# urbste/MultiCol-SLAM

Hardware: AMD Instinct MI355X
Metric: Mfeatures/s extract+match, 3-cam 754x480 multi-frame (higher is better)
Workload: dtype u8+i32 (images, Hamming) / f64 (omni model)

## Files before the change

### multicol-slam_amd/csrc/mcs_describe.hip

```cpp
#include "mcs_common.h"
#include <type_traits>
#include "mcs_orient.h"

#include <algorithm>
#include <cstdlib>
#include <vector>

namespace mcs {

__constant__ __attribute__((aligned(16))) signed char c_pattern[2048];

template <int NB> struct UPat;
template <> struct UPat<2> { static constexpr int R = 4, RW = 1; };
template <> struct UPat<4> { static constexpr int R = 6, RW = 2; };
template <> struct UPat<8> { static constexpr int R = 9, RW = 5; };
constexpr int kUPatMax = 9 * 64, kUWMax = 5 * 64;
__device__ double2 g_upat[3][kUPatMax];
__device__ double g_uw[3][kUWMax];
__device__ unsigned short g_gidx[3][64 * 16];

template <int NB>
static bool build_unique_pattern(const signed char* pattern, int slot) {
	constexpr int R = UPat<NB>::R, RW = UPat<NB>::RW, NP = 128 * NB;
	std::vector<int> first, mult, ofPoint(NP);
	for (int i = 0; i < NP; ++i) {
		int f = -1;
		for (size_t k = 0; k < first.size(); ++k)
			if (pattern[2 * first[k]] == pattern[2 * i] && pattern[2 * first[k] + 1] == pattern[2 * i + 1]) { f = (int)k; break; }
		if (f < 0) { f = (int)first.size(); first.push_back(i); mult.push_back(0); }
		mult[f]++; ofPoint[i] = f;
	}
	const int nu = (int)first.size(), pad = R * 64 - nu;
	int heavy = 0;
	for (int m : mult) heavy += m >= 2;
	if (pad < 0 || heavy + pad > RW * 64) return false;
	std::vector<int> order;
	for (int k = 0; k < nu; ++k) if (mult[k] >= 2) order.push_back(k);
	for (int k = 0; k < pad; ++k) order.push_back(-1);
	for (int k = 0; k < nu; ++k) if (mult[k] < 2) order.push_back(k);
	std::vector<int> slotOf(nu);
	std::vector<double2> up(kUPatMax, double2{0.0, 0.0});
	std::vector<double> uw(kUWMax, 0.0);
	for (int sidx = 0; sidx < R * 64; ++sidx) {
		const int k = order[sidx], src = first[k < 0 ? 0 : k];
		up[sidx] = double2{(double)pattern[2 * src], (double)pattern[2 * src + 1]};
		if (k >= 0) slotOf[k] = sidx;
		if (sidx < RW * 64) uw[sidx] = k < 0 ? 0.0 : (double)mult[k];
		else if (k < 0 || mult[k] != 1) return false;
	}
	std::vector<unsigned short> gi(64 * 16, 0);
	for (int l = 0; l < 64; ++l)
		for (int i = 0; i < 2 * NB; ++i) gi[l * 2 * NB + i] = (unsigned short)slotOf[ofPoint[2 * ((i >> 1) * 64 + l) + (i & 1)]];
	return hipMemcpyToSymbol(HIP_SYMBOL(g_upat), up.data(), sizeof(double2) * kUPatMax, sizeof(double2) * kUPatMax * slot) == hipSuccess &&
	       hipMemcpyToSymbol(HIP_SYMBOL(g_uw), uw.data(), sizeof(double) * kUWMax, sizeof(double) * kUWMax * slot) == hipSuccess &&
	       hipMemcpyToSymbol(HIP_SYMBOL(g_gidx), gi.data(), sizeof(unsigned short) * 64 * 16, sizeof(unsigned short) * 64 * 16 * slot) == hipSuccess;
}

bool upload_describe_tables(const signed char* pattern) {
	if (!pattern) return false;
	if (hipMemcpyToSymbol(HIP_SYMBOL(c_pattern), pattern, 2048) != hipSuccess) return false;
	return build_unique_pattern<2>(pattern, 0) && build_unique_pattern<4>(pattern, 1) && build_unique_pattern<8>(pattern, 2);
}

__device__ __forceinline__ double recip_refined(double d) {
	const double r0 = __builtin_amdgcn_rcp(d);
	const double r1 = __builtin_fma(r0, __builtin_fma(-d, r0, 1.0), r0);
	return __builtin_fma(r1, __builtin_fma(-d, r1, 1.0), r1);
}
__device__ __forceinline__ double div_shared(double a, double d, double r) {
	const double q0 = a * r;
	return __builtin_fma(__builtin_fma(-d, q0, a), r, q0);
}

__global__ void k_selftest_recip(unsigned long long seed, int n, int* mismatches) {
	const int i = blockIdx.x * blockDim.x + threadIdx.x;
	if (i >= n) return;
	unsigned long long st = seed + 0x9E3779B97F4A7C15ull * (unsigned long long)(i + 1);
	auto next = [&]() { st ^= st >> 12; st ^= st << 25; st ^= st >> 27; return st * 0x2545F4914F6CDD1Dull; };
	auto unit = [&]() { return (double)(next() >> 11) * (1.0 / 9007199254740992.0); };
	const double ed = -14.0 + 19.0 * unit();
	const double d = exp10(ed) * (1.0 + unit());
	double a = (unit() * 2.0 - 1.0) * exp10(-18.0 + 22.0 * unit());
	if ((i & 127) == 0) a = 0.0;
	if ((i & 127) == 1) a = -d;
	if ((i & 127) == 2) a = d;
	const double r = recip_refined(d);
	const double q1 = div_shared(a, d, r), q2 = a / d;
	if (__double_as_longlong(q1) != __double_as_longlong(q2)) atomicAdd(mismatches, 1);
}

void launch_selftest_recip(unsigned long long seed, int n, int* mismatches, hipStream_t s) {
	hipLaunchKernelGGL(k_selftest_recip, dim3((n + 255) / 256), dim3(256), 0, s, seed, n, mismatches);
}

__device__ __forceinline__ double uniform_f64(const double* p) {
	const unsigned lo = __builtin_amdgcn_readfirstlane(reinterpret_cast<const unsigned*>(p)[0]);
	const unsigned hi = __builtin_amdgcn_readfirstlane(reinterpret_cast<const unsigned*>(p)[1]);
	return __hiloint2double((int)hi, (int)lo);
}

__device__ __forceinline__ double horner_d(const double* coeffs, int s, double x) {
	double c[MCS_MAX_POLY];
#pragma unroll
	for (int i = 0; i < MCS_MAX_POLY; ++i) c[i] = coeffs[i];
	double res = 0.0;
#pragma unroll
	for (int i = MCS_MAX_POLY - 1; i >= 0; i--) res = res * x + c[i];
	(void)s;
	return res;
}

__device__ __forceinline__ void world2img(const OcamDev& cam, double x, double y, double z, double& u, double& v) {
	double norm = sqrt(x * x + y * y);
	if (norm == 0.0) norm = 1e-14;
	const double theta = atan(-z / norm);
	const double rho = horner_d(cam.invP, cam.invP_deg, theta);
	const double uu = x / norm * rho;
	const double vv = y / norm * rho;
	u = uu * cam.c + vv * cam.d + cam.u0;
	v = uu * cam.e + vv + cam.v0;
}

__device__ __forceinline__ void img2world(const OcamDev& cam, double u, double v, double& xo, double& yo, double& zo) {
	const double u_t = u - cam.u0;
	const double v_t = v - cam.v0;
	double x = (u_t - cam.d * v_t) / cam.invAffine;
	double y = (-cam.e * u_t + cam.c * v_t) / cam.invAffine;
	const double X2 = x * x;
	const double Y2 = y * y;
	double z = -horner_d(cam.p, cam.p_deg, sqrt(X2 + Y2));
	double norm = sqrt(X2 + Y2 + z * z);
	xo = x / norm;
	yo = y / norm;
	zo = z / norm;
}

#ifndef MCS_PATCH_R
#define MCS_PATCH_R 21
#endif
constexpr int kPatchR = MCS_PATCH_R, kPatchRows = 2 * kPatchR + 1, kPatchDw = (kPatchRows + 3) / 4, kPatchPitch = 4 * kPatchDw;
constexpr int kPatchBytes = (kPatchRows * kPatchPitch + 15) / 16 * 16;
constexpr int kFPitch = (kPatchRows + 15) / 16 * 16, kFPatchBytes = kPatchRows * kFPitch;

struct Sampler {
	const uint8_t* blur; int bstride;
	const uint8_t* raw; int rstride;
	int w, h;
	const uint8_t* patch; int prow, pcol;
	__device__ __forceinline__ int at(int r, int c) const {
		const unsigned pr = (unsigned)(r - prow), pc = (unsigned)(c - pcol);
		if (pr < (unsigned)kPatchRows && pc < (unsigned)kPatchRows) return patch[pr * kPatchPitch + pc];
		if ((unsigned)r < (unsigned)h && (unsigned)c < (unsigned)w) return blur[(size_t)r * bstride + c];
		r = r < -kEdge ? -kEdge : (r > h + kEdge - 1 ? h + kEdge - 1 : r);
		c = c < -kEdge ? -kEdge : (c > w + kEdge - 1 ? w + kEdge - 1 : c);
		r = r < 0 ? -r : (r >= h ? 2 * (h - 1) - r : r);
		c = c < 0 ? -c : (c >= w ? 2 * (w - 1) - c : c);
		return raw[(size_t)r * rstride + c];
	}
	__device__ __forceinline__ void pair(int row, int col, int dy0, int dx0, int dy1, int dx1, int& t0, int& t1) const {
		const unsigned r0 = (unsigned)(dy0 + kPatchR), c0 = (unsigned)(dx0 + kPatchR), r1 = (unsigned)(dy1 + kPatchR), c1 = (unsigned)(dx1 + kPatchR);
		const bool inside = max(max(r0, c0), max(r1, c1)) < (unsigned)kPatchRows;
		if (!__any(!inside)) {
			t0 = patch[r0 * kPatchPitch + c0];
			t1 = patch[r1 * kPatchPitch + c1];
		} else {
			t0 = at(row + dy0, col + dx0);
			t1 = at(row + dy1, col + dx1);
		}
	}
};

#ifndef MCS_ABLATE
#define MCS_ABLATE 0
#endif
__host__ __device__ constexpr int pat_doubles(int npoints) { return 2 * npoints + 2; }
__host__ __device__ constexpr int coord_bytes(int mode, int npoints) { return mode == 0 ? 0 : pat_doubles(npoints) * 8; }

constexpr int kPatchTrips = (kPatchRows * kPatchDw + 63) / 64;
struct KeyPt {
	int img, out, level, row, col;
	float angle;
	double rayx, rayy, rayz;
	Sampler sm;
};

__device__ __forceinline__ void find_slot(const PyrDesc& d, const int* selCount, int s, int& level, int& pos, int& total) {
	total = 0; level = -1; pos = 0;
	for (int l = 0; l < d.nlevels; ++l) {
		const int c = selCount[l];
		if (s >= total && s < total + c) { level = l; pos = s - total; }
		total += c;
	}
}

__device__ __forceinline__ void patch_load(const uint8_t* blur, int bstride, int row, int col, uint32_t (&pv)[kPatchTrips]) {
	const int lane = threadIdx.x & 63;
	const uint8_t* bp = blur + (size_t)(row - kPatchR) * bstride + (col - kPatchR);
#pragma unroll
	for (int t = 0; t < kPatchTrips; ++t) {
		const int i = min(lane + 64 * t, kPatchRows * kPatchDw - 1);
		const int r = i / kPatchDw, k = i - r * kPatchDw;
		__builtin_memcpy(&pv[t], bp + (size_t)r * bstride + 4 * k, 4);
	}
}
__device__ __forceinline__ void patch_store(uint8_t* patch, const uint32_t (&pv)[kPatchTrips]) {
	const int lane = threadIdx.x & 63;
#pragma unroll
	for (int t = 0; t < kPatchTrips; ++t) {
		const int i = min(lane + 64 * t, kPatchRows * kPatchDw - 1);
		const int r = i / kPatchDw, k = i - r * kPatchDw;
		*reinterpret_cast<uint32_t*>(&patch[r * kPatchPitch + 4 * k]) = pv[t];
	}
}

// ... 388 lines not shown
#pragma unroll
	for (int o = 32; o > 0; o >>= 1) v += __shfl_xor(v, o);
	return v;
}

template <int CTRL>
__device__ __forceinline__ double dpp_f64(double v) {
	const int vl = __double2loint(v), vh = __double2hiint(v);
	const int lo = __builtin_amdgcn_update_dpp(0, vl, CTRL, 0xF, 0xF, true);
	const int hi = __builtin_amdgcn_update_dpp(0, vh, CTRL, 0xF, 0xF, true);
	return __hiloint2double(hi, lo);
}
__device__ __forceinline__ void wave_sum2_f64(double sx, double sy, double& totx, double& toty) {
	const auto l = __builtin_amdgcn_permlane32_swap(__double2loint(sx), __double2loint(sy), false, false);
	const auto h = __builtin_amdgcn_permlane32_swap(__double2hiint(sx), __double2hiint(sy), false, false);
	double z = __hiloint2double((int)h[0], (int)l[0]) + __hiloint2double((int)h[1], (int)l[1]);
	const auto l2 = __builtin_amdgcn_permlane16_swap(__double2loint(z), __double2loint(z), false, false);
	const auto h2 = __builtin_amdgcn_permlane16_swap(__double2hiint(z), __double2hiint(z), false, false);
	z = __hiloint2double((int)h2[0], (int)l2[0]) + __hiloint2double((int)h2[1], (int)l2[1]);
	z += dpp_f64<0x128>(z);
	z += dpp_f64<0x124>(z);
	z += dpp_f64<0x122>(z);
	z += dpp_f64<0x121>(z);
	totx = __hiloint2double(__builtin_amdgcn_readlane(__double2hiint(z), 0), __builtin_amdgcn_readlane(__double2loint(z), 0));
	toty = __hiloint2double(__builtin_amdgcn_readlane(__double2hiint(z), 32), __builtin_amdgcn_readlane(__double2loint(z), 32));
}

struct FastCam { double c, d, e; };
template <class Tab>
__device__ __forceinline__ void fast_w2i(const FastCam& C, Tab tab, double xr, double yr, double& u, double& v, unsigned& top) {
	const double s = __builtin_fma(xr, xr, yr * yr);
	const unsigned hi = (unsigned)__double2hiint(s), lo = (unsigned)__double2loint(s);
	const unsigned idx = (hi >> (20 - kGM)) - (unsigned)((1023 + kGE0) << kGM);
	top = max(top, idx);
	unsigned row = idx < (unsigned)kGRows ? idx : (unsigned)(kGRows - 1);
	if (MCS_FAST_ABLATE & 16) row = 0;
	const double frac = __hiloint2double((int)((hi & ((1u << (20 - kGM)) - 1u)) | 0x3FF00000u), (int)lo);
	const double tau = frac - (1.0 + 1.0 / (double)(2 << kGM));
	typedef double f64x2 __attribute__((ext_vector_type(2)));
	typedef float f32x4 __attribute__((ext_vector_type(4)));
	const auto rowp = reinterpret_cast<const uint8_t*>(tab) + row * (unsigned)kGDevRowBytes;
	const f64x2 g01 = *reinterpret_cast<const f64x2*>(rowp), g23 = *reinterpret_cast<const f64x2*>(rowp + 16);
	const f32x4 g46 = *reinterpret_cast<const f32x4*>(rowp + 32);
	const float tf = (float)tau;
	const float tl = __builtin_fmaf(__builtin_fmaf(g46.z, tf, g46.y), tf, g46.x);
	double G = __builtin_fma((double)tl, tau, g23.y);
	G = __builtin_fma(G, tau, g23.x);
	G = __builtin_fma(G, tau, g01.y);
	G = __builtin_fma(G, tau, g01.x);
	const double uu = xr * G, vv = yr * G;
	u = __builtin_fma(uu, C.c, vv * C.d);
	v = __builtin_fma(uu, C.e, vv);
}

template <int MODE>
__global__ __launch_bounds__(256) void k_orient_b(ExtractBuffers b, int wavesPerImage, int nslots) {
	const int gw = blockIdx.x * 256 + threadIdx.x;
	if (gw >= nslots) return;
	KpAuxSoA A; A.carve(b.aux, nslots);
	const PyrDesc& d = *b.desc;
	const int img = gw / wavesPerImage, s = gw - img * wavesPerImage;
	int total, level, pos;
	find_slot(d, b.selCount + (size_t)img * d.nlevels, s, level, pos, total);
	if (s == 0) {
		b.nkp[img] = total < d.kpCap ? total : d.kpCap;
		if (total > d.kpCap) atomicExch(b.status, MCS_ERR_CAPACITY);
	}
	if (level < 0 || s >= d.kpCap) { A.lvl[gw] = -1; return; }
	const LevelInfo& L = d.lv[level];
	const size_t si = (size_t)img * d.selPerImage + L.selBase + pos;
	const uint32_t rec = b.sel[si];
	const float angle = b.selAngle[si];
	const int col = (int)(rec & 0xFFF) + kMinBorder, row = (int)((rec >> 12) & 0xFFF) + kMinBorder;
	float pxf = (float)col, pyf = (float)row;
	if (level != 0) { pxf = pxf * L.scale; pyf = pyf * L.scale; }
	mcs_keypoint kp;
	kp.x = pxf; kp.y = pyf; kp.size = L.kpSize; kp.angle = angle; kp.response = (float)(rec >> 24); kp.octave = level; kp.class_id = -1;
	b.kps[(size_t)img * d.kpCap + s] = kp;
	A.rc[gw] = row | (col << 16);
	A.poff[gw] = (unsigned)(L.off + (size_t)(row - kPatchR) * L.stride + (col - kPatchR));
	const int lvlWord = level | (L.stride << 16);
	if constexpr (MODE == 0) {
		if (b.cams && b.rays) {
			double rx, ry, rz;
			img2world(b.cams[img], (double)pxf, (double)pyf, rx, ry, rz);
			double* rp = b.rays + ((size_t)img * d.kpCap + s) * 3;
			rp[0] = rx; rp[1] = ry; rp[2] = rz;
		}
		const float DEG2RADf = (float)3.1415926535897932384626433832795 / 180.f;
		const double a0 = (double)(angle * DEG2RADf);
		double* D = A.d8 + gw;
		D[(size_t)2 * nslots] = cos(a0); D[(size_t)3 * nslots] = sin(a0);
		A.lvl[gw] = lvlWord;
		return;
	}
	const OcamDev& cam = b.cams[img];
	double rayx, rayy, rayz;
	img2world(cam, (double)pxf, (double)pyf, rayx, rayy, rayz);
	if (b.rays) {
		double* rp = b.rays + ((size_t)img * d.kpCap + s) * 3;
		rp[0] = rayx; rp[1] = rayy; rp[2] = rayz;
	}
	double ukx = 0.0, uky = 0.0;
	if (d.undistort) {
		const double p0 = cam.p[0];
		ukx = -rayx / rayz * p0;
		uky = -rayy / rayz * p0;
	}
	double* D8 = A.d8 + gw;
	const size_t S = (size_t)nslots;
	D8[0] = ukx; D8[S] = uky;
	const double n2 = ukx * ukx + uky * uky;
	if (cam.fastOk == 0 || !(n2 < 1.0e300)) {
		A.lvl[gw] = lvlWord | kAuxExact;
		b.preList[atomicAdd(b.preCount, 1)] = (uint32_t)gw;
		return;
	}
	A.lvl[gw] = lvlWord;
	double ang[3] = {0.0, 0.0, 0.0};
	if (MODE == 1) {
		const float DEG2RADf = (float)3.1415926535897932384626433832795 / 180.f;
		ang[0] = (double)(angle * DEG2RADf);
	} else {
		const float RHOf = 180.0f / 3.1415926535897932384626f;
		const double RHOd = 180.0 / 3.1415926535897932384626433832795028841971693993;
		const double rot = 20.0 / RHOd;
		ang[0] = (double)(angle / RHOf);
		ang[1] = ang[0] + rot; ang[2] = ang[0] - rot;
	}
#pragma unroll
	for (int k = 0; k < (MODE == 2 ? 3 : 1); ++k) {
		double sn, cs;
		sincos(ang[k], &sn, &cs);
		D8[(2 + 2 * k) * S] = cs; D8[(3 + 2 * k) * S] = sn;
	}
}

#ifndef MCS_FAST_WAVES_PER_EU
#define MCS_FAST_WAVES_PER_EU 4
#endif
#ifndef MCS_FAST_BLOCKS
#define MCS_FAST_BLOCKS (4096 / MCS_FAST_WAVES)
#endif
constexpr int kFastBlocks = MCS_FAST_BLOCKS;
static_assert(kSlotAlign % kFastWaves == 0, "a group's keypoint slots must belong to one image");

struct UTabs {
	const double2* upat; const double* uw; const uint32_t* gidx;
	uint8_t* vals;
};
__host__ __device__ constexpr size_t upat_bytes(int nb) { return (size_t)(nb == 2 ? 4 : nb == 4 ? 6 : 9) * 64 * sizeof(double2); }
__host__ __device__ constexpr size_t uw_bytes(int nb) { return (size_t)(nb == 2 ? 1 : nb == 4 ? 2 : 5) * 64 * sizeof(double); }
__host__ __device__ constexpr size_t gidx_bytes(int nb) { return (size_t)64 * 2 * nb * sizeof(unsigned short); }
__host__ __device__ constexpr size_t uvals_bytes(int nb) { return (size_t)(nb == 2 ? 4 : nb == 4 ? 6 : 9) * 64; }

template <int MODE, int NB, class Ahead>
__device__ __forceinline__ bool fast_keypoint_u(const ExtractBuffers& b, const FastCam& C, const double* tabLds, const uint8_t* patch,
                                                double ukx, double uky, const double (&axc)[3], const double (&ays)[3], const UTabs& T,
                                                unsigned long long (&bitsMain)[NB], unsigned long long (&agree)[NB], Ahead&& ahead) {
	constexpr int NP = 128 * NB, R = UPat<NB>::R, RW = UPat<NB>::RW;
	const double kFix = 1572864.5;
	const unsigned kHiPatch = 0x4137F000u + 4096u - (unsigned)kPatchR;
	const unsigned guardUnits = (unsigned)__builtin_ceil(b.guardEps * 4294967296.0);
	const double gAdd = (double)guardUnits * (1.0 / 4294967296.0);
#pragma unroll
	for (int j = 0; j < NB; ++j) { bitsMain[j] = 0ull; agree[j] = ~0ull; }
	constexpr int npat = MODE == 2 ? 3 : 1;
	typedef double f64x2 __attribute__((ext_vector_type(2)));
	typedef const __attribute__((address_space(3))) f64x2 lds_f64x2;
	typedef const __attribute__((address_space(3))) double lds_f64;
	typedef const __attribute__((address_space(3))) uint32_t lds_u32;
	typedef __attribute__((address_space(3))) uint8_t lds_u8;
	typedef const __attribute__((address_space(3))) uint8_t lds_cu8;
	unsigned pdo = (unsigned)(uintptr_t)(lds_f64x2*)T.upat, pwo = (unsigned)(uintptr_t)(lds_f64*)T.uw, pgo = (unsigned)(uintptr_t)(lds_u32*)T.gidx;
	unsigned pvo = (unsigned)(uintptr_t)(lds_u8*)T.vals, plo = (unsigned)(uintptr_t)(lds_cu8*)patch;
	int lane = threadIdx.x & 63;
	asm volatile("" : "+v"(pdo), "+v"(pwo), "+v"(pgo), "+s"(pvo), "+s"(plo), "+v"(lane));
	lds_f64x2* const pd = (lds_f64x2*)(uintptr_t)pdo;
	lds_f64* const pw = (lds_f64*)(uintptr_t)pwo;
	lds_u32* const pg = (lds_u32*)(uintptr_t)pgo;
	lds_u8* const pv = (lds_u8*)(uintptr_t)pvo;
	lds_cu8* const pvr = (lds_cu8*)(uintptr_t)pvo;
	lds_cu8* const pl = (lds_cu8*)(uintptr_t)plo;
	unsigned top = 0, minlo = 0xFFFFFFFFu, maxrc = 0;
	bool bad = false;
#pragma unroll
	for (int pat = 0; pat < npat; ++pat) {
		const double ax = axc[pat], ay = ays[pat];
		double u[R], v[R];
		double sumx = 0.0, sumy = 0.0;
#pragma unroll
		for (int t = 0; t < R; ++t) {
			const f64x2 p = pd[64 * t];
			if (pat == 0 && t == 0) ahead();
			const double xr = __builtin_fma(p.x, ax, __builtin_fma(-p.y, ay, ukx));
			const double yr = __builtin_fma(p.x, ay, __builtin_fma(p.y, ax, uky));
			if (MCS_FAST_ABLATE & 2) { u[t] = xr; v[t] = yr; } else fast_w2i(C, tabLds, xr, yr, u[t], v[t], top);
			if (t < RW) { const double w = pw[64 * t]; sumx = __builtin_fma(w, u[t], sumx); sumy = __builtin_fma(w, v[t], sumy); }
			else { sumx += u[t]; sumy += v[t]; }
			constexpr int kFence = R > 6 ? 2 : MCS_FAST_FENCE;
			if ((t & (kFence - 1)) == kFence - 1) __builtin_amdgcn_sched_barrier(0);
		}
		double totx, toty;
		wave_sum2_f64(sumx, sumy, totx, toty);
		const double meanX = totx * (1.0 / (double)NP), meanY = toty * (1.0 / (double)NP);
		bad |= !(fabs(meanX) < 16384.0) || !(fabs(meanY) < 16384.0);
		const double cmx = (kFix - meanX) + gAdd, cmy = (kFix - meanY) + gAdd;
		if (R > 6) __builtin_amdgcn_sched_barrier(0);
		int val[R];
#pragma unroll
		for (int t = 0; t < R; ++t) {
			const double yx = u[t] + cmx, yy = v[t] + cmy;
			const unsigned pc = (unsigned)__double2hiint(yx) - kHiPatch, pr = (unsigned)__double2hiint(yy) - kHiPatch;
			if (!(MCS_FAST_ABLATE & 4)) minlo = min(minlo, min((unsigned)__double2loint(yx), (unsigned)__double2loint(yy)));
			maxrc = max(maxrc, max(pr, pc));
			static_assert(kFPitch == 48, "the shift-add form is for a pitch of 48");
			unsigned off16 = (pr << 4) + pc;
			asm volatile("" : "+v"(off16));
			const unsigned offRaw = (pr << 5) + off16;
			const unsigned off = min(offRaw, (unsigned)(kFPatchBytes - 1));
			val[t] = (MCS_FAST_ABLATE & 1) ? (int)off : (int)pl[off];
		}
#pragma unroll
		for (int t = 0; t < R; ++t) pv[64 * t + lane] = (uint8_t)val[t];
		__builtin_amdgcn_fence(__ATOMIC_RELEASE, "wavefront");
#pragma unroll
		for (int j = 0; j < NB; ++j) {
			const uint32_t g = pg[j];
			const int t0 = pvr[g & 0xFFFFu], t1 = pvr[g >> 16];
			const unsigned long long bits = __ballot(t0 < t1);
			if (pat == 0) bitsMain[j] = bits;
			else agree[j] &= ~(bits ^ bitsMain[j]);
		}
		__builtin_amdgcn_fence(__ATOMIC_ACQUIRE, "wavefront");
		if (R > 6) { if (__any(bad | (top >= (unsigned)kGRows) | (minlo < 2u * guardUnits) | (maxrc >= (unsigned)kPatchRows))) return false; }
	}
	bad |= top >= (unsigned)kGRows;
	if (!(MCS_FAST_ABLATE & 4)) bad |= minlo < 2u * guardUnits;
	bad |= maxrc >= (unsigned)kPatchRows;
	return !__any(bad);
}

constexpr int kFastPatchBufs = 2;
constexpr int kMailDwords = 32, kMailBytes = 2 * kMailDwords * 4;
constexpr int kMailCam = 19, kMailUsed = 26;
__host__ __device__ constexpr size_t fast_wave_lds(int nb) { return (size_t)kFastPatchBufs * kFPatchBytes + kMailBytes + uvals_bytes(nb); }
__host__ __device__ constexpr size_t fast_pat_bytes(int nb) { return upat_bytes(nb) + uw_bytes(nb) + gidx_bytes(nb); }

__device__ __forceinline__ unsigned lds_addr(const void* p) { return (unsigned)(uintptr_t)(const __attribute__((address_space(3))) void*)p; }
__device__ __forceinline__ void dma16(const void* g, unsigned ldsBase) {
	asm volatile("s_mov_b32 m0, %1\n\ts_nop 0\n\tglobal_load_lds_dwordx4 %0, off" ::"v"(g), "s"(ldsBase) : "memory", "m0");
}
__device__ __forceinline__ void dma4(const void* g, unsigned ldsBase) {
	asm volatile("s_mov_b32 m0, %1\n\ts_nop 0\n\tglobal_load_lds_dword %0, off" ::"v"(g), "s"(ldsBase) : "memory", "m0");
}
__device__ __forceinline__ void patch_request(const uint8_t* origin, int bstride, uint8_t* patch) {
	int lane = threadIdx.x & 63;
	asm volatile("" : "+v"(lane));
	constexpr int perRow = kFPitch / 16, total = kPatchRows * perRow;
#pragma unroll
	for (int t = 0; t * 64 < total; ++t) {
		const int i = lane + 64 * t;
		const int r = i / perRow, k = i - r * perRow;
		if (64 * (t + 1) <= total || i < total) dma16(origin + (size_t)r * bstride + 16 * k, __builtin_amdgcn_readfirstlane(lds_addr(patch) + 1024 * t));
	}
}
__device__ __forceinline__ void record_request(const KpAuxSoA& A, const OcamDev* cams, int gw, int img, uint32_t* mail) {
	int lane = threadIdx.x & 63;
	asm volatile("" : "+v"(lane));
	const size_t S = (size_t)A.slots;
	const uint32_t* src;
	if (lane < 3) src = reinterpret_cast<const uint32_t*>(A.lvl) + (size_t)lane * S + gw;
	else if (lane < kMailCam) src = reinterpret_cast<const uint32_t*>(A.d8 + (size_t)((lane - 3) >> 1) * S + gw) + ((lane - 3) & 1);
	else if (lane == kMailCam) src = reinterpret_cast<const uint32_t*>(&cams[img].tabIdx);
	else src = reinterpret_cast<const uint32_t*>(&cams[img].c) + (lane - kMailCam - 1);
	if (lane < kMailUsed) dma4(src, __builtin_amdgcn_readfirstlane(lds_addr(mail)));
}
static_assert(offsetof(OcamDev, c) == 0 && offsetof(OcamDev, d) == 8 && offsetof(OcamDev, e) == 16, "record_request reads c, d, e as six consecutive words");

struct FastKp {
	int lvl, rc; unsigned poff; int tabIdx;
	double d8[8]; FastCam C;
	__device__ __forceinline__ bool usable() const { return lvl >= 0 && !(lvl & kAuxExact); }
};
__device__ __forceinline__ int rfl(uint32_t v) { return __builtin_amdgcn_readfirstlane((int)v); }
__device__ __forceinline__ double rfl2(uint32_t lo, uint32_t hi) { return __hiloint2double(rfl(hi), rfl(lo)); }
__device__ __forceinline__ FastKp mail_read(const uint32_t* mail) {
	uint4 q[7];
#pragma unroll
	for (int i = 0; i < 7; ++i) q[i] = reinterpret_cast<const uint4*>(mail)[i];
	const uint32_t* w = reinterpret_cast<const uint32_t*>(q);
	FastKp r;
	r.lvl = rfl(w[0]); r.rc = rfl(w[1]); r.poff = (unsigned)rfl(w[2]); r.tabIdx = rfl(w[kMailCam]);
#pragma unroll
	for (int i = 0; i < 8; ++i) r.d8[i] = rfl2(w[3 + 2 * i], w[4 + 2 * i]);
	r.C.c = rfl2(w[20], w[21]); r.C.d = rfl2(w[22], w[23]); r.C.e = rfl2(w[24], w[25]);
	return r;
}

template <int MODE, int NB>
__attribute__((amdgpu_waves_per_eu(MCS_FAST_WAVES_PER_EU, MCS_FAST_WAVES_PER_EU)))
__global__ __launch_bounds__(64 * kFastWaves) void k_describe_fast(ExtractBuffers b, int wavesPerImage, int nslots, int groupsPerBlock) {
	extern __shared__ __attribute__((aligned(16))) double lds[];
	static_assert(MODE == 1 || MODE == 2, "the fast pass is for the distorted patterns");
	const int wave = __builtin_amdgcn_readfirstlane(threadIdx.x >> 6);
	constexpr size_t kFastWaveLds = fast_wave_lds(NB);
	double2* const patLds = reinterpret_cast<double2*>(reinterpret_cast<uint8_t*>(lds) + kGDevDoubles * sizeof(double));
	uint8_t* const waveLds = reinterpret_cast<uint8_t*>(patLds) + fast_pat_bytes(NB) + (size_t)wave * kFastWaveLds;
	uint32_t* const mailBase = reinterpret_cast<uint32_t*>(waveLds + kFastPatchBufs * kFPatchBytes);
	constexpr int kSlot = NB == 2 ? 0 : NB == 4 ? 1 : 2;
	double* const uwLds = reinterpret_cast<double*>(reinterpret_cast<uint8_t*>(patLds) + upat_bytes(NB));
	uint32_t* const gidxLds = reinterpret_cast<uint32_t*>(reinterpret_cast<uint8_t*>(uwLds) + uw_bytes(NB));
	for (int i = threadIdx.x; i < UPat<NB>::R * 64; i += 64 * kFastWaves) patLds[i] = g_upat[kSlot][i];
	for (int i = threadIdx.x; i < UPat<NB>::RW * 64; i += 64 * kFastWaves) uwLds[i] = g_uw[kSlot][i];
	for (int i = threadIdx.x; i < 64 * NB; i += 64 * kFastWaves) gidxLds[i] = reinterpret_cast<const uint32_t*>(g_gidx[kSlot])[i];
	double* const tabLds = lds;
	const PyrDesc& d = *b.desc;
	KpAuxSoA A; A.carve(b.aux, nslots);
	const int ngroups = nslots / kFastWaves;
	const int nb = (int)gridDim.x, perXcd = (nb + kNumXCD - 1) / kNumXCD;
	const int logical = nb % kNumXCD == 0 ? ((int)blockIdx.x % kNumXCD) * perXcd + (int)blockIdx.x / kNumXCD : (int)blockIdx.x;
	const size_t pyrBytes = d.pyrBytes;
	int curTab = -1;
	auto slot_of = [&](int kk) { const int g = kk * nb + logical; return kk < groupsPerBlock && g < ngroups ? g * kFastWaves + wave : -1; };
	auto ask_record = [&](int kk) { const int gw = slot_of(kk); if (gw >= 0) record_request(A, b.cams, gw, gw / wavesPerImage, mailBase + (kk & 1) * kMailDwords); };
	auto ask_patch = [&](const FastKp& r, int kk) {
		const int gw = slot_of(kk);
		if (gw < 0 || !r.usable()) return;
		patch_request(b.blur + (size_t)(gw / wavesPerImage) * pyrBytes + r.poff, (int)((unsigned)r.lvl >> 16), waveLds + (kk & 1) * kFPatchBytes);
	};
	ask_record(0);
	asm volatile("s_waitcnt vmcnt(0)" ::: "memory");
	FastKp nxt = mail_read(mailBase);
	if (slot_of(0) < 0) nxt.lvl = -1;
	ask_patch(nxt, 0);
	ask_record(1);
	FastKp cur = nxt;
	auto advance = [&](int k) {
		asm volatile("s_waitcnt vmcnt(0)" ::: "memory");
		cur = nxt;
		nxt = mail_read(mailBase + (k & 1) * kMailDwords);
		if (slot_of(k + 2) < 0) nxt.lvl = -1;
	};
#pragma unroll 1
	for (int k = 0; k < groupsPerBlock; ++k) {
		const int g = k * nb + logical;
		if (g >= ngroups) break;
		const int base = g * kFastWaves;
		const int bimg = base / wavesPerImage;
		const int gwu = base + wave;
		int lane = threadIdx.x & 63;
		asm volatile("" : "+v"(lane));
		advance(k - 1);
		const FastKp me = cur;
		auto ahead = [&]() {
			ask_patch(nxt, k + 1);
			ask_record(k + 2);
		};
		const int tabIdx = me.tabIdx;
		uint8_t* const patchLds = waveLds + (k & 1) * kFPatchBytes;
		if (tabIdx != curTab) {
			if (curTab >= 0) __syncthreads();
			if (!(MCS_FAST_ABLATE & 8)) {
				const double2* gt = reinterpret_cast<const double2*>(b.gTab + (size_t)tabIdx * kGDevDoubles);
				constexpr int n2 = kGDevDoubles / 2, trips = (n2 + 64 * kFastWaves - 1) / (64 * kFastWaves);
				double2 tv[trips];
#pragma unroll
				for (int t = 0; t < trips; ++t) { const int i = t * 64 * kFastWaves + (int)threadIdx.x; tv[t] = i < n2 ? gt[i] : double2{0.0, 0.0}; }
#pragma unroll
				for (int t = 0; t < trips; ++t) { const int i = t * 64 * kFastWaves + (int)threadIdx.x; if (i < n2) reinterpret_cast<double2*>(tabLds)[i] = tv[t]; }
			}
			__syncthreads();
			curTab = tabIdx;
		}
		if (!me.usable()) { ahead(); continue; }
		const FastCam C = me.C;
		const double ukx = me.d8[0], uky = me.d8[1];
		double axc[3], ays[3];
#pragma unroll
		for (int q = 0; q < 3; ++q) { axc[q] = me.d8[2 + 2 * q]; ays[q] = me.d8[3 + 2 * q]; }
		unsigned long long bitsMain[NB], agree[NB];
		UTabs T;
		T.upat = patLds + lane; T.uw = uwLds + lane; T.gidx = gidxLds + lane * NB; T.vals = waveLds + kFastPatchBufs * kFPatchBytes + kMailBytes;
		const bool ok = fast_keypoint_u<MODE, NB>(b, C, tabLds, patchLds, ukx, uky, axc, ays, T, bitsMain, agree, ahead);
		if (lane == 0) {
			if (!ok) { const int at = atomicAdd(b.fbCount, 1); b.fbList[at] = (uint32_t)gwu; }
			else {
				const int out = gwu - bimg * wavesPerImage;
				uint8_t* dout = b.out_desc + ((size_t)bimg * b.outImgPitch + out) * b.outRowStride;
				uint8_t* mout = b.out_mask + ((size_t)bimg * b.outImgPitch + out) * b.outRowStride;
#pragma unroll
				for (int j = 0; j < NB; ++j) {
					*reinterpret_cast<unsigned long long*>(dout + 8 * j) = bitsMain[j];
					*reinterpret_cast<unsigned long long*>(mout + 8 * j) = MODE == 2 ? agree[j] : 0ull;
				}
			}
		}
	}
}

__global__ void k_selftest_fast_model(const OcamDev* camp, const double* tab, unsigned long long seed, int n, int width, int height, unsigned long long* maxDiff) {
	const int i = blockIdx.x * blockDim.x + threadIdx.x;
	if (i >= n) return;
	const OcamDev& cam = *camp;
	unsigned long long st = seed + 0x9E3779B97F4A7C15ull * (unsigned long long)(i + 1);
	auto next = [&]() { st ^= st >> 12; st ^= st << 25; st ^= st >> 27; return st * 0x2545F4914F6CDD1Dull; };
	auto unit = [&]() { return (double)(next() >> 11) * (1.0 / 9007199254740992.0); };
	const double px = unit() * width, py = unit() * height;
	double rx, ry, rz;
	img2world(cam, px, py, rx, ry, rz);
	const double p0 = cam.p[0];
	const double xr = -rx / rz * p0 + (unit() * 64.0 - 32.0), yr = -ry / rz * p0 + (unit() * 64.0 - 32.0);
	double ue, ve;
	world2img(cam, xr, yr, -p0, ue, ve);
	FastCam C;
	C.c = cam.c; C.d = cam.d; C.e = cam.e;
	double uf, vf;
	unsigned top = 0;
	fast_w2i(C, tab, xr, yr, uf, vf, top);
	if (top >= (unsigned)kGRows) return;
	double diff = fmax(fabs(uf + cam.u0 - ue), fabs(vf + cam.v0 - ve));
	if (!(diff == diff)) diff = 1e300;
	atomicMax(maxDiff, (unsigned long long)__double_as_longlong(diff));
}

void launch_selftest_fast_model(const OcamDev* cam, const double* tab, unsigned long long seed, int n, int width, int height, unsigned long long* maxDiff, hipStream_t s) {
	hipLaunchKernelGGL(k_selftest_fast_model, dim3((n + 255) / 256), dim3(256), 0, s, cam, tab, seed, n, width, height, maxDiff);
}

template <int NB>
__global__ __launch_bounds__(256) void k_describe_orb(ExtractBuffers b, int wavesPerImage, int nslots) {
	extern __shared__ double orb_lds[];
	const PyrDesc& d = *b.desc;
	const int lane = threadIdx.x & 63, wave = threadIdx.x >> 6;
	const int gw = __builtin_amdgcn_readfirstlane((int)blockIdx.x * 4 + wave);
	if (gw >= nslots) return;
	KpAuxSoA A; A.carve(b.aux, nslots);
	const int lw = __builtin_amdgcn_readfirstlane(A.lvl[gw]);
	if (lw < 0) return;
	const int level = lw & 0xFF;
	const int rc = __builtin_amdgcn_readfirstlane(A.rc[gw]);
	const int row = rc & 0xFFFF, col = (int)((unsigned)rc >> 16);
	const int img = gw / wavesPerImage, out = gw - img * wavesPerImage;
	const double ax = uniform_f64(A.d8 + (size_t)2 * nslots + gw), ay = uniform_f64(A.d8 + (size_t)3 * nslots + gw);
	const LevelInfo& L = d.lv[level];
	uint8_t* patch = reinterpret_cast<uint8_t*>(orb_lds) + (size_t)wave * kPatchBytes;
	Sampler sm = {};
	int rstride;
	sm.raw = level_ptr(b, d, img, level, &rstride); sm.rstride = rstride; sm.w = L.w; sm.h = L.h;
	sm.blur = b.blur + (size_t)img * d.pyrBytes + L.off; sm.bstride = L.stride;
	uint32_t pv[kPatchTrips];
	patch_load(sm.blur, sm.bstride, row, col, pv);
	patch_store(patch, pv);
	sm.patch = patch; sm.prow = row - kPatchR; sm.pcol = col - kPatchR;
	uint8_t* dout = b.out_desc + ((size_t)img * b.outImgPitch + out) * b.outRowStride;
	uint8_t* mout = b.out_mask + ((size_t)img * b.outImgPitch + out) * b.outRowStride;
	double tie = 0.0;
#pragma unroll
	for (int j = 0; j < NB; ++j) {
		const int k = j * 64 + lane;
		const double x0 = c_pattern[4 * k], y0 = c_pattern[4 * k + 1], x1 = c_pattern[4 * k + 2], y1 = c_pattern[4 * k + 3];
		const double fx0 = x0 * ax - y0 * ay, fy0 = x0 * ay + y0 * ax, fx1 = x1 * ax - y1 * ay, fy1 = x1 * ay + y1 * ax;
		const int ix0 = __double2int_rn(fx0), iy0 = __double2int_rn(fy0);
		const int ix1 = __double2int_rn(fx1), iy1 = __double2int_rn(fy1);
		tie = fmax(fmax(tie, fmax(tie_frac(fx0), tie_frac(fy0))), fmax(tie_frac(fx1), tie_frac(fy1)));
		int t0, t1;
		sm.pair(row, col, iy0, ix0, iy1, ix1, t0, t1);
		const unsigned long long bits = __ballot(t0 < t1);
		if (lane == 0) {
			*reinterpret_cast<unsigned long long*>(dout + 8 * j) = bits;
			*reinterpret_cast<unsigned long long*>(mout + 8 * j) = 0ull;
		}
	}
	tie_commit(b, gw, tie);
}

template <int MODE, int NB>
static void launch_fast_passes(const ExtractBuffers& b, int nimg, int wavesPerImage, size_t listLds, hipStream_t s) {
	const int nslots = nimg * wavesPerImage, ngroups = nslots / kFastWaves, lblocks = std::min(nslots, 2048);
	const int groupsPerBlock = std::max(1, (ngroups + kFastBlocks - 1) / kFastBlocks);
	int fblocks = (ngroups + groupsPerBlock - 1) / groupsPerBlock;
	if (fblocks >= kNumXCD) fblocks = (fblocks + kNumXCD - 1) / kNumXCD * kNumXCD;
	const size_t fLds = (size_t)kFastWaves * fast_wave_lds(NB) + kGDevDoubles * sizeof(double) + fast_pat_bytes(NB);
	hipLaunchKernelGGL((k_orient_b<MODE>), dim3((nslots + 255) / 256), dim3(256), 0, s, b, wavesPerImage, nslots);
	hipStream_t ps = b.sideStream ? b.sideStream : s;
	if (b.sideStream) { (void)hipEventRecord(b.evDescFork, s); (void)hipStreamWaitEvent(ps, b.evDescFork, 0); }
	hipLaunchKernelGGL((k_describe_list<MODE, NB>), dim3(lblocks), dim3(64), listLds, ps, b, wavesPerImage, b.preCount, b.preList);
	if (b.sideStream) (void)hipEventRecord(b.evDescJoin, ps);
	if (fLds > 65536) (void)hipFuncSetAttribute(reinterpret_cast<const void*>(&k_describe_fast<MODE, NB>), hipFuncAttributeMaxDynamicSharedMemorySize, (int)fLds);
	if (b.evFastA) (void)hipEventRecord(b.evFastA, s);
	hipLaunchKernelGGL((k_describe_fast<MODE, NB>), dim3(fblocks), dim3(64 * kFastWaves), fLds, s, b, wavesPerImage, nslots, groupsPerBlock);
	if (b.evFastB) (void)hipEventRecord(b.evFastB, s);
	static const bool split = !(getenv("MCS_LIST_SPLIT") && atoi(getenv("MCS_LIST_SPLIT")) == 0);
	typedef SplitGeom<MODE, NB> SG;
	if (split) hipLaunchKernelGGL((k_describe_list_split<MODE, NB>), dim3(std::min(nslots, 512)), dim3(64 * SG::WAVES), SG::lds_bytes(), s, b, wavesPerImage, b.fbCount, b.fbList);
	else hipLaunchKernelGGL((k_describe_list<MODE, NB>), dim3(lblocks), dim3(64), listLds, s, b, wavesPerImage, b.fbCount, b.fbList);
	if (b.sideStream) (void)hipStreamWaitEvent(s, b.evDescJoin, 0);
}

template <int MODE>
static void launch_mode(const ExtractBuffers& b, const PyrDesc& hd, int nimg, hipStream_t s) {
	const int wpb = MODE == 0 ? 4 : 1;
	const int wavesPerImage = (hd.kpCap + kSlotAlign - 1) / kSlotAlign * kSlotAlign;
	const int blocks = nimg * wavesPerImage / wpb;
	const size_t ldsBytes = (size_t)wpb * (coord_bytes(MODE, hd.npoints) + kPatchBytes);
	const int nb = hd.descSize / 8;
	if constexpr (MODE != 0) {
		if (b.describeMode == 0) {
			if (nb == 2) launch_fast_passes<MODE, 2>(b, nimg, wavesPerImage, ldsBytes, s);
			else if (nb == 4) launch_fast_passes<MODE, 4>(b, nimg, wavesPerImage, ldsBytes, s);
			else launch_fast_passes<MODE, 8>(b, nimg, wavesPerImage, ldsBytes, s);
			return;
		}
	}
	if constexpr (MODE == 0) {
		static const bool orbSplit = !(getenv("MCS_ORB_SPLIT") && atoi(getenv("MCS_ORB_SPLIT")) == 0);
		static const bool orbForce = getenv("MCS_ORB_SPLIT") != nullptr;
		if (orbSplit && b.aux && (orbForce || nimg * wavesPerImage >= 8192)) {
			const int nslots = nimg * wavesPerImage;
			hipLaunchKernelGGL((k_orient_b<0>), dim3((nslots + 255) / 256), dim3(256), 0, s, b, wavesPerImage, nslots);
			if (b.evFastA) (void)hipEventRecord(b.evFastA, s);
			if (nb == 2) hipLaunchKernelGGL((k_describe_orb<2>), dim3(blocks), dim3(256), ldsBytes, s, b, wavesPerImage, nslots);
			else if (nb == 4) hipLaunchKernelGGL((k_describe_orb<4>), dim3(blocks), dim3(256), ldsBytes, s, b, wavesPerImage, nslots);
			else hipLaunchKernelGGL((k_describe_orb<8>), dim3(blocks), dim3(256), ldsBytes, s, b, wavesPerImage, nslots);
			if (b.evFastB) (void)hipEventRecord(b.evFastB, s);
			return;
		}
	}
	if (b.evFastA) (void)hipEventRecord(b.evFastA, s);
	if (nb == 2) hipLaunchKernelGGL((k_describe<MODE, 2>), dim3(blocks), dim3(64 * wpb), ldsBytes, s, b, wavesPerImage);
	else if (nb == 4) hipLaunchKernelGGL((k_describe<MODE, 4>), dim3(blocks), dim3(64 * wpb), ldsBytes, s, b, wavesPerImage);
	else if constexpr (MODE == 2) hipLaunchKernelGGL((k_describe_wide<MODE, 8>), dim3(blocks), dim3(64 * wpb), ldsBytes, s, b, wavesPerImage);
	else hipLaunchKernelGGL((k_describe<MODE, 8>), dim3(blocks), dim3(64 * wpb), ldsBytes, s, b, wavesPerImage);
	if (b.evFastB) (void)hipEventRecord(b.evFastB, s);
}

size_t describe_aux_bytes() { return KpAuxSoA::bytes_per_slot(); }

void launch_describe(const ExtractBuffers& b, const PyrDesc& hd, int nimg, hipStream_t s) {
	if (hd.mode == 0) launch_mode<0>(b, hd, nimg, s);
	else if (hd.mode == 1) launch_mode<1>(b, hd, nimg, s);
	else launch_mode<2>(b, hd, nimg, s);
}

}
```

Measured before the change: 141.5.

## Interleave pattern sample values in LDS and add optional bank-aware pattern ordering

```diff
diff --git a/multicol-slam_amd/csrc/mcs_describe.hip b/multicol-slam_amd/csrc/mcs_describe.hip
--- a/multicol-slam_amd/csrc/mcs_describe.hip
+++ b/multicol-slam_amd/csrc/mcs_describe.hip
@@ -1,6 +1,7 @@
 #include "mcs_common.h"
 #include <type_traits>
 #include "mcs_orient.h"
+#include "mcs_upat.h"
 
 #include <algorithm>
 #include <cstdlib>
@@ -20,37 +21,17 @@
 __device__ unsigned short g_gidx[3][64 * 16];
 
 template <int NB>
-static bool build_unique_pattern(const signed char* pattern, int slot) {
-	constexpr int R = UPat<NB>::R, RW = UPat<NB>::RW, NP = 128 * NB;
-	std::vector<int> first, mult, ofPoint(NP);
-	for (int i = 0; i < NP; ++i) {
-		int f = -1;
-		for (size_t k = 0; k < first.size(); ++k)
-			if (pattern[2 * first[k]] == pattern[2 * i] && pattern[2 * first[k] + 1] == pattern[2 * i + 1]) { f = (int)k; break; }
-		if (f < 0) { f = (int)first.size(); first.push_back(i); mult.push_back(0); }
-		mult[f]++; ofPoint[i] = f;
-	}
-	const int nu = (int)first.size(), pad = R * 64 - nu;
-	int heavy = 0;
-	for (int m : mult) heavy += m >= 2;
-	if (pad < 0 || heavy + pad > RW * 64) return false;
-	std::vector<int> order;
-	for (int k = 0; k < nu; ++k) if (mult[k] >= 2) order.push_back(k);
-	for (int k = 0; k < pad; ++k) order.push_back(-1);
-	for (int k = 0; k < nu; ++k) if (mult[k] < 2) order.push_back(k);
-	std::vector<int> slotOf(nu);
+static bool build_unique_pattern(const signed char* pattern, int slot, bool bankAware) {
+	static_assert(UPat<NB>::R * 64 <= kUPatMax && UPat<NB>::RW * 64 <= kUWMax, "table sizes");
+	mcs_upat::Layout L;
+	if (!mcs_upat::build(pattern, NB, bankAware, L) || L.R != UPat<NB>::R || L.RW != UPat<NB>::RW) return false;
 	std::vector<double2> up(kUPatMax, double2{0.0, 0.0});
 	std::vector<double> uw(kUWMax, 0.0);
-	for (int sidx = 0; sidx < R * 64; ++sidx) {
-		const int k = order[sidx], src = first[k < 0 ? 0 : k];
-		up[sidx] = double2{(double)pattern[2 * src], (double)pattern[2 * src + 1]};
-		if (k >= 0) slotOf[k] = sidx;
-		if (sidx < RW * 64) uw[sidx] = k < 0 ? 0.0 : (double)mult[k];
-		else if (k < 0 || mult[k] != 1) return false;
-	}
 	std::vector<unsigned short> gi(64 * 16, 0);
+	for (int sidx = 0; sidx < L.R * 64; ++sidx) up[sidx] = double2{(double)L.x[sidx], (double)L.y[sidx]};
+	std::copy(L.w.begin(), L.w.end(), uw.begin());
 	for (int l = 0; l < 64; ++l)
-		for (int i = 0; i < 2 * NB; ++i) gi[l * 2 * NB + i] = (unsigned short)slotOf[ofPoint[2 * ((i >> 1) * 64 + l) + (i & 1)]];
+		for (int i = 0; i < 2 * NB; ++i) gi[((i >> 1) * 64 + l) * 2 + (i & 1)] = L.gidx[l * 2 * NB + i];
 	return hipMemcpyToSymbol(HIP_SYMBOL(g_upat), up.data(), sizeof(double2) * kUPatMax, sizeof(double2) * kUPatMax * slot) == hipSuccess &&
 	       hipMemcpyToSymbol(HIP_SYMBOL(g_uw), uw.data(), sizeof(double) * kUWMax, sizeof(double) * kUWMax * slot) == hipSuccess &&
 	       hipMemcpyToSymbol(HIP_SYMBOL(g_gidx), gi.data(), sizeof(unsigned short) * 64 * 16, sizeof(unsigned short) * 64 * 16 * slot) == hipSuccess;
@@ -59,7 +40,8 @@
 bool upload_describe_tables(const signed char* pattern) {
 	if (!pattern) return false;
 	if (hipMemcpyToSymbol(HIP_SYMBOL(c_pattern), pattern, 2048) != hipSuccess) return false;
-	return build_unique_pattern<2>(pattern, 0) && build_unique_pattern<4>(pattern, 1) && build_unique_pattern<8>(pattern, 2);
+	static const bool bankAware = getenv("MCS_UPAT_ORDER") && atoi(getenv("MCS_UPAT_ORDER")) != 0;
+	return build_unique_pattern<2>(pattern, 0, bankAware) && build_unique_pattern<4>(pattern, 1, bankAware) && build_unique_pattern<8>(pattern, 2, bankAware);
 }
 
 __device__ __forceinline__ double recip_refined(double d) {
@@ -754,7 +736,7 @@
 __host__ __device__ constexpr size_t upat_bytes(int nb) { return (size_t)(nb == 2 ? 4 : nb == 4 ? 6 : 9) * 64 * sizeof(double2); }
 __host__ __device__ constexpr size_t uw_bytes(int nb) { return (size_t)(nb == 2 ? 1 : nb == 4 ? 2 : 5) * 64 * sizeof(double); }
 __host__ __device__ constexpr size_t gidx_bytes(int nb) { return (size_t)64 * 2 * nb * sizeof(unsigned short); }
-__host__ __device__ constexpr size_t uvals_bytes(int nb) { return (size_t)(nb == 2 ? 4 : nb == 4 ? 6 : 9) * 64; }
+__host__ __device__ constexpr size_t uvals_bytes(int nb) { return (size_t)128 * (((nb == 2 ? 4 : nb == 4 ? 6 : 9) + 1) / 2); }
 
 template <int MODE, int NB, class Ahead>
 __device__ __forceinline__ bool fast_keypoint_u(const ExtractBuffers& b, const FastCam& C, const double* tabLds, const uint8_t* patch,
@@ -776,8 +758,8 @@
 	typedef const __attribute__((address_space(3))) uint8_t lds_cu8;
 	unsigned pdo = (unsigned)(uintptr_t)(lds_f64x2*)T.upat, pwo = (unsigned)(uintptr_t)(lds_f64*)T.uw, pgo = (unsigned)(uintptr_t)(lds_u32*)T.gidx;
 	unsigned pvo = (unsigned)(uintptr_t)(lds_u8*)T.vals, plo = (unsigned)(uintptr_t)(lds_cu8*)patch;
-	int lane = threadIdx.x & 63;
-	asm volatile("" : "+v"(pdo), "+v"(pwo), "+v"(pgo), "+s"(pvo), "+s"(plo), "+v"(lane));
+	int tidv = threadIdx.x;
+	asm volatile("" : "+v"(pdo), "+v"(pwo), "+v"(pgo), "+s"(pvo), "+s"(plo));
 	lds_f64x2* const pd = (lds_f64x2*)(uintptr_t)pdo;
 	lds_f64* const pw = (lds_f64*)(uintptr_t)pwo;
 	lds_u32* const pg = (lds_u32*)(uintptr_t)pgo;
@@ -823,12 +805,14 @@
 			const unsigned off = min(offRaw, (unsigned)(kFPatchBytes - 1));
 			val[t] = (MCS_FAST_ABLATE & 1) ? (int)off : (int)pl[off];
 		}
-#pragma unroll
-		for (int t = 0; t < R; ++t) pv[64 * t + lane] = (uint8_t)val[t];
+		asm volatile("" : "+v"(tidv));
+		const int vlane = 4 * (tidv & 31) + ((tidv >> 5) & 1);
+#pragma unroll
+		for (int t = 0; t < R; ++t) pv[vlane + 2 * (t & 1) + 128 * (t >> 1)] = (uint8_t)val[t];
 		__builtin_amdgcn_fence(__ATOMIC_RELEASE, "wavefront");
 #pragma unroll
 		for (int j = 0; j < NB; ++j) {
-			const uint32_t g = pg[j];
+			const uint32_t g = pg[64 * j];
 			const int t0 = pvr[g & 0xFFFFu], t1 = pvr[g >> 16];
 			const unsigned long long bits = __ballot(t0 < t1);
 			if (pat == 0) bitsMain[j] = bits;
@@ -983,7 +967,7 @@
 		for (int q = 0; q < 3; ++q) { axc[q] = me.d8[2 + 2 * q]; ays[q] = me.d8[3 + 2 * q]; }
 		unsigned long long bitsMain[NB], agree[NB];
 		UTabs T;
-		T.upat = patLds + lane; T.uw = uwLds + lane; T.gidx = gidxLds + lane * NB; T.vals = waveLds + kFastPatchBufs * kFPatchBytes + kMailBytes;
+		T.upat = patLds + lane; T.uw = uwLds + lane; T.gidx = gidxLds + lane; T.vals = waveLds + kFastPatchBufs * kFPatchBytes + kMailBytes;
 		const bool ok = fast_keypoint_u<MODE, NB>(b, C, tabLds, patchLds, ukx, uky, axc, ays, T, bitsMain, agree, ahead);
 		if (lane == 0) {
 			if (!ok) { const int at = atomicAdd(b.fbCount, 1); b.fbList[at] = (uint32_t)gwu; }
@@ -1083,7 +1067,8 @@
 	const int groupsPerBlock = std::max(1, (ngroups + kFastBlocks - 1) / kFastBlocks);
 	int fblocks = (ngroups + groupsPerBlock - 1) / groupsPerBlock;
 	if (fblocks >= kNumXCD) fblocks = (fblocks + kNumXCD - 1) / kNumXCD * kNumXCD;
-	const size_t fLds = (size_t)kFastWaves * fast_wave_lds(NB) + kGDevDoubles * sizeof(double) + fast_pat_bytes(NB);
+	constexpr size_t fLds = (size_t)kFastWaves * fast_wave_lds(NB) + kGDevDoubles * sizeof(double) + fast_pat_bytes(NB);
+	static_assert(fLds <= 160 * 1024 && fast_wave_lds(NB) % 16 == 0, "one workgroup's LDS: a CU has 160 KiB; the patch buffers are written in 16-byte pieces");
 	hipLaunchKernelGGL((k_orient_b<MODE>), dim3((nslots + 255) / 256), dim3(256), 0, s, b, wavesPerImage, nslots);
 	hipStream_t ps = b.sideStream ? b.sideStream : s;
 	if (b.sideStream) { (void)hipEventRecord(b.evDescFork, s); (void)hipStreamWaitEvent(ps, b.evDescFork, 0); }
diff --git a/multicol-slam_amd/csrc/mcs_upat.h b/multicol-slam_amd/csrc/mcs_upat.h
--- /dev/null
+++ b/multicol-slam_amd/csrc/mcs_upat.h
@@ -0,0 +1,245 @@
+#pragma once
+#include <algorithm>
+#include <cmath>
+#include <cstdlib>
+#include <vector>
+
+namespace mcs_upat {
+
+inline int rounds(int nb) { return nb == 2 ? 4 : nb == 4 ? 6 : nb == 8 ? 9 : 0; }
+inline int weighted_rounds(int nb) { return nb == 2 ? 1 : nb == 4 ? 2 : nb == 8 ? 5 : 0; }
+inline int vals_addr(int t, int l) { return 4 * (l & 31) + (l >> 5) + 2 * (t & 1) + 128 * (t >> 1); }
+inline int vals_bytes(int nb) { return 128 * ((rounds(nb) + 1) / 2); }
+constexpr int kPatchR = 21, kPatchPitch = 48;
+
+struct Layout {
+	int nb = 0, R = 0, RW = 0, nu = 0;
+	std::vector<int> order;
+	std::vector<signed char> x, y;
+	std::vector<double> w;
+	std::vector<unsigned short> gidx;
+};
+
+struct Cycles { double patch = 0, vals_read = 0, vals_write = 0; };
+
+namespace detail {
+
+inline int half_depth(const int* dword, const int* key, int n) {
+	int seen[32][32], cnt[32] = {0}, depth = 0;
+	for (int i = 0; i < n; ++i) {
+		const int b = dword[i] & 31;
+		bool dup = false;
+		for (int k = 0; k < cnt[b]; ++k) dup |= seen[b][k] == key[i];
+		if (!dup) { seen[b][cnt[b]++] = key[i]; depth = std::max(depth, cnt[b]); }
+	}
+	return depth;
+}
+
+struct Item { int k, x, y; };
+
+inline void bisect(std::vector<Item>& it, int lo, int hi, int g, std::vector<std::vector<Item>>& out) {
+	if (g == 1) { out.emplace_back(it.begin() + lo, it.begin() + hi); return; }
+	int x0 = 127, x1 = -128, y0 = 127, y1 = -128;
+	for (int i = lo; i < hi; ++i) { x0 = std::min(x0, it[i].x); x1 = std::max(x1, it[i].x); y0 = std::min(y0, it[i].y); y1 = std::max(y1, it[i].y); }
+	const bool byX = x1 - x0 >= y1 - y0;
+	std::sort(it.begin() + lo, it.begin() + hi, [byX](const Item& a, const Item& b) {
+		const int a0 = byX ? a.x : a.y, b0 = byX ? b.x : b.y, a1 = byX ? a.y : a.x, b1 = byX ? b.y : b.x;
+		return a0 != b0 ? a0 < b0 : a1 != b1 ? a1 < b1 : a.k < b.k;
+	});
+	const int n = hi - lo, gl = g / 2, gr = g - gl;
+	const int nl = std::min(32 * gl, std::max(n - 32 * gr, (n * gl + g / 2) / g));
+	bisect(it, lo, lo + nl, gl, out);
+	bisect(it, lo + nl, hi, gr, out);
+}
+
+}
+
+inline Cycles model_cycles(const Layout& L, double angle) {
+	Cycles c;
+	const double ca = std::cos(angle), sa = std::sin(angle);
+	int dw[32], key[32];
+	for (int t = 0; t < L.R; ++t)
+		for (int h = 0; h < 2; ++h) {
+			for (int i = 0; i < 32; ++i) {
+				const int s = t * 64 + h * 32 + i;
+				const int px = (int)std::lrint(L.x[s] * ca - L.y[s] * sa), py = (int)std::lrint(L.x[s] * sa + L.y[s] * ca);
+				const int off = (py + kPatchR) * kPatchPitch + (px + kPatchR);
+				dw[i] = key[i] = off >> 2;
+			}
+			c.patch += detail::half_depth(dw, key, 32);
+			for (int i = 0; i < 32; ++i) { key[i] = vals_addr(t, h * 32 + i); dw[i] = key[i] >> 2; }
+			c.vals_write += detail::half_depth(dw, key, 32);
+		}
+	for (int g = 0; g < 2 * L.nb; ++g)
+		for (int h = 0; h < 2; ++h) {
+			for (int i = 0; i < 32; ++i) dw[i] = key[i] = L.gidx[(h * 32 + i) * 2 * L.nb + g] >> 2;
+			c.vals_read += detail::half_depth(dw, key, 32);
+		}
+	return c;
+}
+
+inline Cycles model_sweep(const Layout& L, int nangles = 64) {
+	Cycles s;
+	for (int a = 0; a < nangles; ++a) {
+		const Cycles c = model_cycles(L, 6.283185307179586 * a / nangles);
+		s.patch += c.patch; s.vals_read += c.vals_read; s.vals_write += c.vals_write;
+	}
+	return s;
+}
+
+inline bool build(const signed char* pattern, int nb, bool bankAware, Layout& L) {
+	const int R = rounds(nb), RW = weighted_rounds(nb), NP = 128 * nb;
+	if (!pattern || R == 0) return false;
+	std::vector<int> first, mult, ofPoint(NP);
+	for (int i = 0; i < NP; ++i) {
+		int f = -1;
+		for (size_t k = 0; k < first.size(); ++k)
+			if (pattern[2 * first[k]] == pattern[2 * i] && pattern[2 * first[k] + 1] == pattern[2 * i + 1]) { f = (int)k; break; }
+		if (f < 0) { f = (int)first.size(); first.push_back(i); mult.push_back(0); }
+		mult[f]++; ofPoint[i] = f;
+	}
+	const int nu = (int)first.size(), pad = R * 64 - nu;
+	int heavy = 0;
+	for (int m : mult) heavy += m >= 2;
+	if (pad < 0 || heavy + pad > RW * 64) return false;
+	auto px = [&](int k) { return (int)pattern[2 * first[k < 0 ? 0 : k]]; };
+	auto py = [&](int k) { return (int)pattern[2 * first[k < 0 ? 0 : k] + 1]; };
+
+	std::vector<int> order;
+	if (!bankAware) {
+		for (int k = 0; k < nu; ++k) if (mult[k] >= 2) order.push_back(k);
+		for (int k = 0; k < pad; ++k) order.push_back(-1);
+		for (int k = 0; k < nu; ++k) if (mult[k] < 2) order.push_back(k);
+	} else {
+		using detail::Item;
+		std::vector<Item> a, b;
+		for (int k = 0; k < nu; ++k) if (mult[k] >= 2) a.push_back(Item{k, px(k), py(k)});
+		for (int k = 0; k < pad; ++k) a.push_back(Item{-1, px(-1), py(-1)});
+		std::vector<std::vector<Item>> groups;
+		detail::bisect(a, 0, (int)a.size(), 2 * RW, groups);
+		std::vector<char> used(nu, 0);
+		for (bool more = true; more;) {
+			more = false;
+			for (auto& g : groups) {
+				if ((int)g.size() >= 32) continue;
+				long sx = 0, sy = 0;
+				for (const Item& it : g) { sx += it.x; sy += it.y; }
+				const int n = std::max(1, (int)g.size());
+				int best = -1; long bestD = 0;
+				for (int k = 0; k < nu; ++k) {
+					if (mult[k] != 1 || used[k]) continue;
+					const long dx = (long)px(k) * n - sx, dy = (long)py(k) * n - sy, d = dx * dx + dy * dy;
+					if (best < 0 || d < bestD) { best = k; bestD = d; }
+				}
+				if (best < 0) return false;
+				used[best] = 1; g.push_back(Item{best, px(best), py(best)});
+				more = true;
+			}
+		}
+		for (int k = 0; k < nu; ++k) if (mult[k] == 1 && !used[k]) b.push_back(Item{k, px(k), py(k)});
+		if ((int)b.size() != (R - RW) * 64) return false;
+		if (R > RW) detail::bisect(b, 0, (int)b.size(), 2 * (R - RW), groups);
+		const int nh = 2 * R, nsets = 4 * nb;
+		std::vector<int> hOf(nu, 0), jOf(nu, 0);
+		std::vector<std::vector<int>> bank(nh, std::vector<int>(32));
+		for (int h = 0; h < nh; ++h)
+			for (int j = 0; j < 32; ++j) { bank[h][j] = j; if (groups[h][j].k >= 0) { hOf[groups[h][j].k] = h; jOf[groups[h][j].k] = j; } }
+		std::vector<std::vector<int>> setPts(nsets), ptSets(nu);
+		for (int g = 0; g < 2 * nb; ++g)
+			for (int l = 0; l < 64; ++l) {
+				const int k = ofPoint[2 * ((g >> 1) * 64 + l) + (g & 1)], s = 2 * g + (l >> 5);
+				setPts[s].push_back(k);
+				if (std::find(ptSets[k].begin(), ptSets[k].end(), s) == ptSets[k].end()) ptSets[k].push_back(s);
+			}
+		auto setCost = [&](int s, unsigned char* cnt) {
+			unsigned char seen[32 * 5] = {0};
+			int depth = 0, extra = 0;
+			for (int b2 = 0; b2 < 32; ++b2) cnt[b2] = 0;
+			for (int i = 0; i < 32; ++i) {
+				const int k = setPts[s][i], h = hOf[k], bnk = bank[h][jOf[k]], d = bnk + 32 * (h >> 2);
+				if (seen[d]) continue;
+				seen[d] = 1;
+				depth = std::max(depth, (int)++cnt[bnk]); extra += cnt[bnk] > 1;
+			}
+			return 1024 * depth + extra;
+		};
+		{
+			std::vector<unsigned char> occ((size_t)nsets * 32, 0);
+			for (int h = 0; h < nh; ++h) {
+				unsigned taken = 0;
+				for (int j = 0; j < 32; ++j) {
+					const int k = groups[h][j].k;
+					int best = -1, bestC = 0;
+					for (int b2 = 0; b2 < 32; ++b2) {
+						if (taken >> b2 & 1) continue;
+						int c = 0;
+						if (k >= 0) for (int s : ptSets[k]) c += __builtin_popcount(occ[(size_t)s * 32 + b2] & ~(1u << (h >> 2)));
+						if (best < 0 || c < bestC) { best = b2; bestC = c; }
+					}
+					bank[h][j] = best; taken |= 1u << best;
+					if (k >= 0) for (int s : ptSets[k]) occ[(size_t)s * 32 + best] |= (unsigned char)(1u << (h >> 2));
+				}
+			}
+		}
+		std::vector<int> cost(nsets);
+		std::vector<unsigned char> cnt((size_t)nsets * 32);
+		for (int s = 0; s < nsets; ++s) cost[s] = setCost(s, &cnt[(size_t)s * 32]);
+		auto crowded = [&](int k, int bnk) {
+			if (k >= 0) for (int s : ptSets[k]) if (cnt[(size_t)s * 32 + bnk] > 1) return true;
+			return false;
+		};
+		constexpr int kPasses = 3;
+		for (int pass = 0, improved = 1; pass < kPasses && improved; ++pass) {
+			improved = 0;
+			for (int h = 0; h < nh; ++h)
+				for (int i = 0; i < 32; ++i)
+					for (int j = 0; j < 32; ++j) {
+						const int ki = groups[h][i].k, kj = groups[h][j].k;
+						if (i == j || !crowded(ki, bank[h][i])) continue;
+						int sets[16], ns = 0, before = 0;
+						for (int k : {ki, kj})
+							if (k >= 0)
+								for (int s : ptSets[k]) {
+									bool have = false;
+									for (int q = 0; q < ns; ++q) have |= sets[q] == s;
+									if (!have && ns < 16) { sets[ns++] = s; before += cost[s]; }
+								}
+						std::swap(bank[h][i], bank[h][j]);
+						int after = 0, c[16];
+						unsigned char cn[16][32];
+						for (int q = 0; q < ns; ++q) { c[q] = setCost(sets[q], cn[q]); after += c[q]; }
+						if (after < before) {
+							for (int q = 0; q < ns; ++q) { cost[sets[q]] = c[q]; std::copy(cn[q], cn[q] + 32, &cnt[(size_t)sets[q] * 32]); }
+							improved = 1;
+						} else std::swap(bank[h][i], bank[h][j]);
+					}
+		}
+		order.assign(R * 64, -1);
+		for (int h = 0; h < nh; ++h)
+			for (int j = 0; j < 32; ++j) order[(h >> 1) * 64 + (h & 1) * 32 + bank[h][j]] = groups[h][j].k;
+	}
+	if ((int)order.size() != R * 64) return false;
+
+	L.nb = nb; L.R = R; L.RW = RW; L.nu = nu;
+	L.order = order;
+	L.x.assign(R * 64, 0); L.y.assign(R * 64, 0); L.w.assign(RW * 64, 0.0); L.gidx.assign(64 * 2 * nb, 0);
+	std::vector<int> slotOf(nu, -1);
+	for (int s = 0; s < R * 64; ++s) {
+		const int k = order[s];
+		L.x[s] = (signed char)px(k); L.y[s] = (signed char)py(k);
+		if (k >= 0) { if (slotOf[k] >= 0) return false; slotOf[k] = s; }
+		if (s < RW * 64) L.w[s] = k < 0 ? 0.0 : (double)mult[k];
+		else if (k < 0 || mult[k] != 1) return false;
+	}
+	for (int l = 0; l < 64; ++l)
+		for (int i = 0; i < 2 * nb; ++i) {
+			const int s = slotOf[ofPoint[2 * ((i >> 1) * 64 + l) + (i & 1)]];
+			if (s < 0) return false;
+			L.gidx[l * 2 * nb + i] = (unsigned short)vals_addr(s >> 6, s & 63);
+		}
+	return true;
+}
+
+}
+
+inline mcs_upat::Cycles upat_model_cycles(const mcs_upat::Layout& L, double angle) { return mcs_upat::model_cycles(L, angle); }
```

New measurement: 141.8 (median of 3 runs). No clear change (+0.2%).
